# edshkim98/LocalDiffusion-Hallucination

Hardware: AMD Instinct MI355X
Metric: local patches/sec (256^2, T=1000) (higher is better)
Workload: dtype bf16; 1 GPU; cfg3: 8 local patches (vertical band masks) of one 3x256x256 image per GPU, 4-stage dim-32 conditional UNet (12.1M params), DDPM T=1000, pred_x0, sigmoid schedule; patches_per_gpu=8, parallelism=patch-sharded x1, one all-gather per sample, step_graph_replay=True, whole_batch_graph_flag=False, concurrent_sub_batches=2, weight_split_levels=0

## Files before the change

include/localdiff_hip.h:

```cpp
#ifndef LOCALDIFF_HIP_H
#define LOCALDIFF_HIP_H

#include <stddef.h>
#include <stdint.h>

#ifdef __cplusplus
extern "C" {
#endif

#define LD_OK 0
#define LD_EINVAL (-1)
#define LD_EHIP (-2)
#define LD_ETIMEOUT (-3)

#define LD_F32 0
#define LD_BF16 1
#define LD_F16 2

#define LD_STAT_STRIPES 16

#define LD_ACT_NONE 0
#define LD_ACT_SILU 1
#define LD_ACT_RELU 2

// ... 38 lines not shown
  int32_t gn_groups;
  int32_t act;
  const float* film;
  int32_t film_tstride;
  int32_t film_bstride;
} ld_src;

typedef struct ld_conv3x3_args {
  ld_src src[2];
  int32_t nsrc;
  const void* weight;
  const float* bias;
  void* out;
  double* out_stats;
  int32_t out_groups;
  int32_t B, H, W, Cout;
  const int32_t* t_ptr;
  int32_t dtype;
  const void* addend;
  int32_t weight_terms;
  const void* side_weight;
  const float* side_bias;
  void* side_out;
} ld_conv3x3_args;
int ld_conv3x3(const ld_conv3x3_args* args, void* stream);

#define LD_EPI_PLAIN 0
#define LD_EPI_QKV_LINEAR 1
#define LD_EPI_QKV_FULL 2
#define LD_EPI_RMS_RES 3
#define LD_EPI_RES 4
#define LD_EPI_GN_TAIL 5
typedef struct ld_conv1x1_args {
  ld_src src[2];
  int32_t nsrc;
  int32_t unshuffle;
  int32_t rms_in;
  const void* weight;
  int64_t weight_bstride;
  const float* bias;
  int32_t epilogue;
  int32_t hidden;
  float q_scale;
  const float* g2;
  const void* residual;
  ld_src gn_tail;
// ... 429 lines not shown
```

localdiffusion-hallucination_amd/_cabi.py:

```python
import ctypes as C
import os

from .tuning import lib_override_path

_HERE = os.path.dirname(os.path.abspath(__file__))

LIB_PATH = lib_override_path() or os.path.join(_HERE, "csrc", "liblocaldiff_hip.so")

LD_F32, LD_BF16, LD_F16 = 0, 1, 2
ACT_NONE, ACT_SILU, ACT_RELU = 0, 1, 2
EPI_PLAIN, EPI_QKV_LINEAR, EPI_QKV_FULL, EPI_RMS_RES, EPI_RES, EPI_GN_TAIL = 0, 1, 2, 3, 4, 5
OBJ = {"pred_x0": 0, "pred_noise": 1, "pred_v": 2}
SCHED_COLS = 8
STAT_STRIPES = 16
COUNTER_CONV3X3_C32, COUNTER_CONV3X3_GENERIC, COUNTER_CONV3X3_S32 = 0, 1, 2
SEG_SRC_PLAIN, SEG_SRC_POOL, SEG_SRC_CAT_D2S = 0, 1, 2
CLF_PLAIN, CLF_HALVE, CLF_AFFINE = 0, 1, 2

vp, i32, i64, u64, f32 = C.c_void_p, C.c_int32, C.c_int64, C.c_uint64, C.c_float


class Src(C.Structure):
    _fields_ = [("data", vp), ("C", i32), ("pix_stride", i32), ("upsample", i32), ("gn_stats", vp),
                ("gn_gamma", vp), ("gn_beta", vp), ("gn_groups", i32), ("act", i32), ("film", vp),
                ("film_tstride", i32), ("film_bstride", i32)]


class Conv3x3Args(C.Structure):
    _fields_ = [("src", Src * 2), ("nsrc", i32), ("weight", vp), ("bias", vp), ("out", vp),
                ("out_stats", vp), ("out_groups", i32), ("B", i32), ("H", i32), ("W", i32),
                ("Cout", i32), ("t_ptr", vp), ("dtype", i32), ("addend", vp), ("weight_terms", i32),
                ("side_weight", vp), ("side_bias", vp), ("side_out", vp)]


class Conv1x1Args(C.Structure):
    _fields_ = [("src", Src * 2), ("nsrc", i32), ("unshuffle", i32), ("rms_in", i32), ("weight", vp),
                ("weight_bstride", i64), ("bias", vp), ("epilogue", i32), ("hidden", i32),
                ("q_scale", f32), ("g2", vp), ("residual", vp), ("gn_tail", Src), ("out", vp), ("kmax_out", vp), ("B", i32), ("H", i32),
                ("W", i32), ("Cout", i32), ("dtype", i32), ("weight_terms", i32)]


class GnApplyArgs(C.Structure):
    _fields_ = [("a", Src), ("b", Src), ("final_act", i32), ("pool", i32), ("out", vp), ("B", i32),
                ("H", i32), ("W", i32), ("t_ptr", vp), ("dtype", i32)]


class StepBeginArgs(C.Structure):
    _fields_ = [("zero_a", vp), ("bytes_a", C.c_size_t), ("zero_b", vp), ("bytes_b", C.c_size_t), ("t_ptr", vp), ("delta", i32),
                ("idx_ptr", vp), ("t_table", vp), ("film_rows", vp), ("row_floats", i32), ("film_cur", vp)]


class SegConvArgs(C.Structure):
    _fields_ = [("src0", vp), ("src1", vp), ("C0", i32), ("C1", i32), ("mode", i32), ("ksize", i32), ("weight", vp),
                ("scale", vp), ("shift", vp), ("relu", i32), ("out", vp), ("B", i32), ("H", i32), ("W", i32),
                ("Cout", i32), ("dtype", i32)]
# ... 278 lines not shown
```

localdiffusion-hallucination_amd/csrc/conv3x3.hip:

```cpp
#include "common.hip.h"
#include <stdlib.h>

int ld_conv3x3_c32_try(const ld_conv3x3_args* p, hipStream_t st);
int ld_conv3x3_s32_try(const ld_conv3x3_args* p, hipStream_t st);
#ifdef LD_DEBUG_VARIANTS
int ld_conv3x3_ksplit_try(const ld_conv3x3_args* p, hipStream_t st);
int ld_conv3x3_ring_try(const ld_conv3x3_args* p, hipStream_t st);
#endif

#include "conv3x3_body.hip.h"

namespace {

#ifdef LD_DEBUG_VARIANTS
int g_span_shape[1024][5];
#endif

template <typename T, int MT, int NW, bool DEEP, int DBG, bool SK = false, bool RAW = false, bool SIDE = false>
int launch_dbg(const Conv3Dev& a, hipStream_t st) {
  constexpr int TR = 4 * NW, HR = TR + 2, HC = 18;
  constexpr int NPIXP = (HR * HC + 15) / 16 * 16;
  const int ctot = a.s[0].C + (a.nsrc > 1 ? a.s[1].C : 0);
  const size_t lds = (SK ? 2 : 1) * (4 * NPIXP * 16 + (9 + (SIDE ? 1 : 0)) * MT * 1024) + 2 * ctot * sizeof(float) + 4 * 2 * 16 * MT * sizeof(double);
  Conv3Dev d = a;
  d.tiles_x = (a.W + 15) / 16;
  const int tiles_y = (a.H + TR - 1) / TR;
  dim3 grid(d.tiles_x * tiles_y, a.Cout / (16 * MT), a.B);
  if (lds > 65536) LD_HIP(ld_allow_lds(conv3x3_kernel<T, MT, NW, DEEP, DBG, SK, RAW, SIDE>, lds));
  LD_LAUNCH((conv3x3_kernel<T, MT, NW, DEEP, DBG, SK, RAW, SIDE>), grid, dim3(SK ? 512 : 256), lds, st, d.s[0].data, d.w, d.H, d.W, d.tiles_x,
            d.s[0].C, d.s[0].ld, d.s[0].ups, d.nsrc, d.wsplit, d.Cout, d);
  LD_LAUNCH_CHECK("conv3x3");
  return LD_OK;
}

template <typename T, int MT, int NW, bool DEEP>
int launch(const Conv3Dev& a, hipStream_t st) {
#ifdef LD_DEBUG_VARIANTS
  if constexpr (std::is_same<T, bf16>::value && !DEEP) {
    switch (a.dbg & 255) {
      case 1: return launch_dbg<T, MT, NW, DEEP, 1>(a, st);
      case 2: return launch_dbg<T, MT, NW, DEEP, 2>(a, st);
      case 3: return launch_dbg<T, MT, NW, DEEP, 3>(a, st);
      case 4: return launch_dbg<T, MT, NW, DEEP, 4>(a, st);
      case 7: return launch_dbg<T, MT, NW, DEEP, 7>(a, st);
      case 8: return launch_dbg<T, MT, NW, DEEP, 8>(a, st);
      case 12: return launch_dbg<T, MT, NW, DEEP, 12>(a, st);
      case 15: return launch_dbg<T, MT, NW, DEEP, 15>(a, st);
      case 64: return launch_dbg<T, MT, NW, DEEP, 64>(a, st);
      case 128:
        if (!a.s[0].stats && !(a.nsrc > 1 && a.s[1].stats)) return launch_dbg<T, MT, NW, DEEP, 128, false, true>(a, st);
        return launch_dbg<T, MT, NW, DEEP, 128>(a, st);
      default: break;
    }
  }
#endif
  if constexpr (!DEEP) {
    const bool raw = !a.s[0].stats && !(a.nsrc > 1 && a.s[1].stats);
    if (raw && ld_tuning().conv_raw) return launch_dbg<T, MT, NW, DEEP, 0, false, true>(a, st);
  }
  return launch_dbg<T, MT, NW, DEEP, 0>(a, st);
}

template <typename T>
int dispatch(const Conv3Dev& a, hipStream_t st) {
#ifdef LD_DEBUG_VARIANTS
  static const int force_mt = getenv("LD_CONV_MT") ? atoi(getenv("LD_CONV_MT")) : 0;
  static const int force_nw = getenv("LD_CONV_NW") ? atoi(getenv("LD_CONV_NW")) : 0;
#else
  constexpr int force_mt = 0, force_nw = 0;
#endif
  const LdTuning& tn = ld_tuning();
  bool mt4 = (a.Cout % 64) == 0;
  const long mt4_min = tn.conv_mt4_min_wgs;
  if (mt4 && (long)((a.W + 15) / 16) * ((a.H + 7) / 8) * (a.Cout / 64) * a.B < mt4_min) mt4 = false;
  const long blocks16 = (long)((a.W + 15) / 16) * ((a.H + 15) / 16) * (a.Cout / (mt4 ? 64 : 32)) * a.B;
  const long big_min = tn.conv_big_min;
  bool big = blocks16 >= big_min && a.H >= 16 && !mt4;
  if (mt4 && a.H >= 16 && blocks16 >= tn.conv_big4_min) big = true;
  if (force_mt == 2) mt4 = false;
  if (force_mt == 4 && (a.Cout % 64) == 0) mt4 = true;
  if (force_nw == 2) big = false;
  if (force_nw == 4) big = true;
#ifdef LD_DEBUG_VARIANTS
  static const int force_deep = getenv("LD_CONV_DEEP") ? atoi(getenv("LD_CONV_DEEP")) : -1;
#else
  constexpr int force_deep = -1;
#endif
  const int ck = sizeof(T) == 4 ? 16 : 32;
  const int nch = (a.s[0].C + (a.nsrc > 1 ? a.s[1].C : 0)) / ck;
  const long wg = (long)((a.W + 15) / 16) * ((a.H + 7) / 8) * (a.Cout / (mt4 ? 64 : 32)) * a.B;
  bool deep = false;
  if (force_deep >= 0) deep = force_deep != 0;
  if constexpr (sizeof(T) == 2) {
    if (a.w2) {
      if (mt4) return launch_dbg<T, 4, 2, false, 0, false, true, true>(a, st);
      return launch_dbg<T, 2, 2, false, 0, false, true, true>(a, st);
    }
  }
  const int force_sk = (int)tn.conv_sk;
  const long sk_max_wgs = tn.conv_sk_max_wgs;
  bool sk = force_sk >= 1 && sizeof(T) == 2 && !big && !deep && ((nch >= 8 && wg <= sk_max_wgs) || force_sk == 2);
  if constexpr (sizeof(T) == 2) {
    if (sk) return mt4 ? launch_dbg<T, 4, 2, false, 0, true>(a, st) : launch_dbg<T, 2, 2, false, 0, true>(a, st);
  }
#ifdef LD_DEBUG_VARIANTS
  if (deep && !big) return mt4 ? launch<T, 4, 2, true>(a, st) : launch<T, 2, 2, true>(a, st);
#endif
  (void)deep;
  if (mt4) return big ? launch<T, 4, 4, false>(a, st) : launch<T, 4, 2, false>(a, st);
  return big ? launch<T, 2, 4, false>(a, st) : launch<T, 2, 2, false>(a, st);
}

}

#ifdef LD_DEBUG_VARIANTS
extern "C" int ld_debug_conv_spans(unsigned long long* spans, int* shapes) {
  LD_HIP(hipDeviceSynchronize());
// ... 23 lines not shown
    LD_REQUIRE(S.data != nullptr, "ld_conv3x3: src[%d] null", s);
    LD_REQUIRE(S.C > 0 && S.C % 32 == 0, "ld_conv3x3: src[%d].C=%d must be a multiple of 32", s, S.C);
    if (S.upsample) LD_REQUIRE(p->H % 2 == 0 && p->W % 2 == 0, "ld_conv3x3: upsample needs even H,W");
    if (S.gn_stats) {
      LD_REQUIRE(S.gn_groups <= 16, "ld_conv3x3: src[%d] gn_groups %d > 16 (the stripe reduction uses 16 lanes per group)", s, S.gn_groups);
      LD_REQUIRE(S.gn_gamma && S.gn_beta && S.gn_groups > 0 && S.C % S.gn_groups == 0,
                 "ld_conv3x3: src[%d] GroupNorm prologue incomplete", s);
    }
    a.s[s] = to_dev(S);
  }
  if (p->nsrc == 1) a.s[1] = a.s[0];
  if (p->out_stats) {
    LD_REQUIRE(p->out_groups > 0 && p->Cout % p->out_groups == 0 && (p->Cout / p->out_groups) <= 32,
               "ld_conv3x3: out_groups %d incompatible with Cout %d", p->out_groups, p->Cout);
  }
  a.w = p->weight; a.bias = p->bias; a.out = p->out; a.ostats = p->out_stats;
  a.ogroups = p->out_groups > 0 ? p->out_groups : 1;
  a.B = p->B; a.H = p->H; a.W = p->W; a.Cout = p->Cout; a.t_ptr = p->t_ptr; a.tiles_x = 0;
  a.addend = p->addend;
  a.w2 = p->side_weight; a.bias2 = p->side_bias; a.out2 = p->side_out;
  if (p->side_weight) {
    LD_REQUIRE(ld_dtype_16(p->dtype), "ld_conv3x3: the side (res_conv) output needs 16-bit storage");
    LD_REQUIRE(p->side_bias && p->side_out, "ld_conv3x3: side_weight without side_bias / side_out");
    LD_REQUIRE(p->weight_terms != 2 && !p->addend, "ld_conv3x3: the side output does not combine with two-term weights or an addend");
    for (int s = 0; s < p->nsrc; ++s)
      LD_REQUIRE(!p->src[s].gn_stats && !p->src[s].upsample, "ld_conv3x3: the side output needs raw, un-resampled sources (a ResnetBlock's block1)");
  }
  LD_REQUIRE(p->weight_terms >= 0 && p->weight_terms <= 2 && !(p->weight_terms == 2 && !ld_dtype_16(p->dtype)),
             "ld_conv3x3: weight_terms %d (2 needs 16-bit storage)", p->weight_terms);
  a.wsplit = p->weight_terms == 2 ? 1 : 0;
  a.dbg = 0;
#ifdef LD_DEBUG_VARIANTS
  static const int dbg = getenv("LD_CONV_DEBUG") ? atoi(getenv("LD_CONV_DEBUG")) : 0;
  a.dbg = dbg;
  if (dbg == 128) {
    static int calls = 0;
    const int slot = calls++ & 1023;
    g_span_shape[slot][0] = p->B; g_span_shape[slot][1] = p->H; g_span_shape[slot][2] = p->W;
    g_span_shape[slot][3] = p->src[0].C + (p->nsrc > 1 ? p->src[1].C : 0); g_span_shape[slot][4] = p->Cout;
    a.dbg = 128 | (slot << 8);
  }
#endif
  hipStream_t st = reinterpret_cast<hipStream_t>(stream);
  if (p->side_weight) {
    ld_count(LD_COUNTER_CONV3X3_GENERIC);
    return LD_DISPATCH16(p->dtype, dispatch<T>(a, st));
  }
  if (p->weight_terms != 2) {
    const int rc = ld_conv3x3_c32_try(p, st);
    if (rc != 0) return rc < 0 ? rc : LD_OK;
  }
  {
    const int rc = ld_conv3x3_s32_try(p, st);
    if (rc != 0) return rc < 0 ? rc : LD_OK;
  }
#ifdef LD_DEBUG_VARIANTS
  {
    const int rc = ld_conv3x3_ring_try(p, st);
    if (rc != 0) return rc < 0 ? rc : LD_OK;
  }
  static const int ksplit = getenv("LD_CONV_KSPLIT") ? atoi(getenv("LD_CONV_KSPLIT")) : 0;
  if (ksplit && p->weight_terms != 2) {
    const int rc = ld_conv3x3_ksplit_try(p, st);
    if (rc != 0) return rc < 0 ? rc : LD_OK;
  }
#endif
  ld_count(LD_COUNTER_CONV3X3_GENERIC);
  return LD_DISPATCH(p->dtype, dispatch<T>(a, st));
}
// ... 1 lines not shown
```

localdiffusion-hallucination_amd/csrc/conv3x3_body.hip.h:

```cpp
#pragma once
#include "common.hip.h"

namespace {

struct Conv3Dev {
  SrcDev s[2];
  const void* w;
  const float* bias;
  void* out;
  double* ostats;
  const int* t_ptr;
  const void* addend;
  const void* w2;
  const float* bias2;
  void* out2;
  int nsrc;
  int ogroups;
  int B, H, W, Cout;
  int tiles_x;
  int wsplit;
  int dbg;
};

__device__ unsigned long long g_conv_trace[24];
__device__ unsigned long long g_conv_span[1024][2];
#define TR_STAMP(k) do { if ((DBG & 64) && tracing) tr_t[k] = __builtin_readcyclecounter(); } while (0)

typedef const Conv3Dev __attribute__((address_space(4)))* Conv3KernargPtr;
template <typename T, int MT, int NW, bool DEEP, int DBG, bool SK = false, bool RAW = false, bool SIDE = false>
__device__ __forceinline__ void conv3x3_tile(const Conv3Dev& head, Conv3KernargPtr rest, const int bx, const int by, const int bz,
                                             const int gdx, const int gdz, char* smem) {
  Conv3Dev a = head;
  constexpr int E = DT<T>::E, CK = DT<T>::CK;
  constexpr int TR = 4 * NW, TC = 16, HR = TR + 2, HC = TC + 2;
  constexpr int NPIX = HR * HC, NPIXP = (NPIX + 15) / 16 * 16, PLANE = NPIXP * 16;
  constexpr int ITER = (NPIXP + 63) / 64;
  constexpr int UNITS = 9 * MT * 64, WU = (UNITS + 255) / 256;
  constexpr bool P = DT<T>::precise;

  static_assert(!SIDE || (RAW && !SK && !DEEP && MT * NW < 16 && sizeof(T) == 2), "SIDE: RAW 16-bit launches of the small register tiles");
  constexpr int STAGE = 4 * PLANE + (9 + (SIDE ? 1 : 0)) * MT * 1024;
  const int half = SK ? (int)(threadIdx.x >> 8) : 0;
  char* s_x = smem + half * STAGE;
  char* s_w = s_x + 4 * PLANE;
  char* s_w2 = s_w + 9 * MT * 1024;
  float* s_coef = reinterpret_cast<float*>(smem + (SK ? 2 : 1) * STAGE);
  double* s_stat;

  const int tid = threadIdx.x & 255, lane = tid & 63, wv = tid >> 6, px = lane & 15, kq = lane >> 4;
  unsigned long long tr_t[24] = {0};
  const bool tracing = (DBG & 64) && threadIdx.x == 0 && bz == gdz / 2 && by == 0 &&
                       bx == (gdx * 5) / 8;
  TR_STAMP(0);
  if ((DBG & 128) && threadIdx.x == 0 && bx == 0 && by == 0 && bz == 0)
    g_conv_span[(a.dbg >> 8) & 1023][0] = __builtin_amdgcn_s_memrealtime();
  const int b = bz, m0 = by * MT;
  int ty_, tx_;
  tile_of(bx, a.tiles_x, gdx / a.tiles_x, ty_, tx_);
  const int ty0 = ty_ * TR, tx0 = tx_ * TC;
  const int H = a.H, W = a.W;
  const int nch0 = a.s[0].C / CK;
  const int ws = a.wsplit;
  int nch = 0;
// ... 106 lines not shown
        }
        *reinterpret_cast<uint4*>(s_x + kq * PLANE + q * 16) = raw;
      }
    }
  };

  TR_STAMP(1);
  if constexpr (SK) { if (half < nch) issue_loads(half, hxA, wxA, std::false_type{}); }
  else issue_loads(0, hxA, wxA, std::true_type{});
  TR_STAMP(2);
  if (rest) {
    Conv3KernargPtr pr = rest;
    asm volatile("" : "+s"(pr));
    a.s[1].data = pr->s[1].data; a.s[1].stats = pr->s[1].stats; a.s[1].gamma = pr->s[1].gamma; a.s[1].beta = pr->s[1].beta;
    a.s[1].film = pr->s[1].film; a.s[1].C = pr->s[1].C; a.s[1].ld = pr->s[1].ld; a.s[1].ups = pr->s[1].ups;
    a.s[1].groups = pr->s[1].groups; a.s[1].act = pr->s[1].act; a.s[1].film_tstride = pr->s[1].film_tstride;
    a.s[1].film_bstride = pr->s[1].film_bstride;
    a.s[0].stats = pr->s[0].stats; a.s[0].gamma = pr->s[0].gamma; a.s[0].beta = pr->s[0].beta; a.s[0].film = pr->s[0].film;
    a.s[0].groups = pr->s[0].groups; a.s[0].act = pr->s[0].act; a.s[0].film_tstride = pr->s[0].film_tstride;
    a.s[0].film_bstride = pr->s[0].film_bstride;
    a.bias = pr->bias; a.out = pr->out; a.ostats = pr->ostats; a.t_ptr = pr->t_ptr; a.addend = pr->addend;
    a.ogroups = pr->ogroups; a.B = pr->B; a.dbg = pr->dbg;
    if constexpr (SIDE) { a.w2 = pr->w2; a.bias2 = pr->bias2; a.out2 = pr->out2; }
  }
  if constexpr (!SK) second_source();
  {
    const int c1 = a.nsrc > 1 ? a.s[1].C : 0;
    nch = (nch0 + c1 / CK) << ws;
    s_stat = reinterpret_cast<double*>(s_coef + 2 * (a.s[0].C + c1));
  }
  asm volatile("" ::"s"(a.bias), "s"(a.out), "s"(a.ostats), "s"(a.ogroups), "s"(a.addend), "s"(a.s[1].C), "s"(a.s[1].ld), "s"(a.s[1].ups),
               "s"(a.s[1].data), "s"(a.s[0].stats), "s"(a.s[0].gamma), "s"(a.s[0].beta), "s"(a.s[0].film), "s"(a.s[0].groups), "s"(a.s[0].act));
  float4 bias[MT];
#pragma unroll
  for (int m = 0; m < MT; ++m) bias[m] = *reinterpret_cast<const float4*>(a.bias + (m0 + m) * 16 + kq * 4);
  float4 bias2[SIDE ? MT : 1];
  if constexpr (SIDE) {
    asm volatile("" ::"s"(a.w2), "s"(a.bias2), "s"(a.out2));
    if (tid < MT * 64) wx2 = *reinterpret_cast<const uint4*>(reinterpret_cast<const char*>(a.w2) + (long)m0 * 1024 + tid * 16);
#pragma unroll
    for (int m = 0; m < MT; ++m) bias2[m] = *reinterpret_cast<const float4*>(a.bias2 + (m0 + m) * 16 + kq * 4);
  }

  {
    const bool any = !RAW && (a.s[0].stats != nullptr || (a.nsrc > 1 && a.s[1].stats != nullptr));
    if (any) {
// ... 160 lines not shown
        compute();
      }
    }
  }

  const int gx = tx0 + px;
  const long obase = (((long)b * H + ty0) * W + tx0) * a.Cout + m0 * 16;
  char* outb = reinterpret_cast<char*>(a.out) + obase * (long)sizeof(T);
  const char* addb = reinterpret_cast<const char*>(a.addend) + obase * (long)sizeof(T);
  const unsigned lane_off = (__umul24(__umul24(wv * NW, W) + px, a.Cout) + kq * 4) * (unsigned)sizeof(T);
  const unsigned row_off = __umul24(W, a.Cout) * (unsigned)sizeof(T);
  float ssum[MT][4], ssq[MT][4];
#pragma unroll
  for (int m = 0; m < MT; ++m)
#pragma unroll
    for (int r = 0; r < 4; ++r) ssum[m][r] = ssq[m][r] = 0.f;
#pragma unroll
  for (int m = 0; m < MT; ++m) asm volatile("" ::"v"(bias[m].x), "v"(bias[m].y), "v"(bias[m].z), "v"(bias[m].w));
  if constexpr (SIDE) {
#pragma unroll
    for (int m = 0; m < MT; ++m) asm volatile("" ::"v"(bias2[m].x), "v"(bias2[m].y), "v"(bias2[m].z), "v"(bias2[m].w));
  }
  const bool rows_in = ty0 + TR <= H && tx0 + TC <= W;
  auto emit = [&](auto full_tag) {
    constexpr bool FULL = decltype(full_tag)::value;
    typename Raw4<T>::type ad[FULL ? 1 : MT][FULL ? 1 : NW];
    if constexpr (!FULL) {
      if (a.addend) {
#pragma unroll
        for (int m = 0; m < MT; ++m)
#pragma unroll
          for (int j = 0; j < NW; ++j) {
            const int gy = ty0 + wv * NW + j;
            const bool in = rows_in || (gy < H && gx < W);
            const unsigned off = lane_off + j * row_off + m * 16 * (unsigned)sizeof(T);
            ad[m][j] = load4_raw<T>(reinterpret_cast<const T*>(addb + (in ? off : 0u)));
          }
#pragma unroll
        for (int m = 0; m < MT; ++m)
#pragma unroll
          for (int j = 0; j < NW; ++j) pin_raw4(ad[m][j]);
      }
    }
    constexpr int MS = sizeof(T) == 2 ? 2 : 1;
    static_assert(MT % 2 == 0, "m-tiles are stored in pairs");
#pragma unroll
// ... 14 lines not shown
              unpack4<T>(ad[m + mm][j], av);
#pragma unroll
              for (int r = 0; r < 4; ++r) v[mm][r] += av[r];
            }
          }
        }
        if constexpr (MS == 2) {
          const uint4 w16 = pair_frag16<T>(v[0], v[1]);
          const unsigned off = lane_off - kq * 4 * (unsigned)sizeof(T) + j * row_off + m * 16 * (unsigned)sizeof(T) + pair_frag16_off(kq);
          if (valid && !(DBG & 8)) store16_out(outb + off, w16);
        } else {
          const unsigned off = lane_off + j * row_off + m * 16 * (unsigned)sizeof(T);
          if (valid && !(DBG & 8)) store4<T>(reinterpret_cast<T*>(outb + off), v[0]);
        }
        if (valid) {
#pragma unroll
          for (int mm = 0; mm < MS; ++mm)
#pragma unroll
            for (int r = 0; r < 4; ++r) { ssum[m + mm][r] += v[mm][r]; ssq[m + mm][r] += v[mm][r] * v[mm][r]; }
        }
      }
    }
  };
  if (rows_in && !a.addend && half == 0) emit(std::true_type{});
  else emit(std::false_type{});
  if constexpr (SIDE) {
    char* out2b = reinterpret_cast<char*>(a.out2) + obase * (long)sizeof(T);
#pragma unroll
    for (int m = 0; m < MT; m += 2) {
#pragma unroll
      for (int j = 0; j < NW; ++j) {
        const int gy = ty0 + wv * NW + j;
        const bool valid = rows_in || (gy < H && gx < W);
        float v[2][4];
#pragma unroll
        for (int mm = 0; mm < 2; ++mm) {
          const float4 bv = bias2[m + mm];
          v[mm][0] = acc2[m + mm][j][0] + bv.x; v[mm][1] = acc2[m + mm][j][1] + bv.y;
          v[mm][2] = acc2[m + mm][j][2] + bv.z; v[mm][3] = acc2[m + mm][j][3] + bv.w;
        }
        const uint4 w16 = pair_frag16<T>(v[0], v[1]);
        const unsigned off = lane_off - kq * 4 * (unsigned)sizeof(T) + j * row_off + m * 16 * (unsigned)sizeof(T) + pair_frag16_off(kq);
        if (valid) store16_out(out2b + off, w16);
      }
    }
  }
  TR_STAMP(9);
  if (a.ostats) {
    __syncthreads();
    TR_STAMP(16);
    const int gs = a.Cout / a.ogroups;
    const int ngrp_blk = (16 * MT) / gs;
    const int stripe = bx % LD_STAT_STRIPES;
    if (!P && (gs & 3) == 0) {
#pragma unroll
      for (int m = 0; m < MT; ++m) {
        const float s1 = wave16_sum((ssum[m][0] + ssum[m][1]) + (ssum[m][2] + ssum[m][3]));
        const float s2 = wave16_sum((ssq[m][0] + ssq[m][1]) + (ssq[m][2] + ssq[m][3]));
        if (px == 0 && half == 0) {
          s_stat[(wv * 2 + 0) * 4 * MT + m * 4 + kq] = (double)s1;
          s_stat[(wv * 2 + 1) * 4 * MT + m * 4 + kq] = (double)s2;
        }
// ... 39 lines not shown
      if (tid < 2 * ngrp_blk && half == 0) {
        const int gi = tid >> 1, k = tid & 1;
        double acc1 = 0.0;
        for (int w4 = 0; w4 < 4; ++w4)
          for (int c = 0; c < gs; ++c) acc1 += s_stat[(w4 * 2 + k) * 16 * MT + gi * gs + c];
        const int g = (m0 * 16) / gs + gi;
        atomicAdd(&a.ostats[(((size_t)b * LD_STAT_STRIPES + stripe) * a.ogroups + g) * 2 + k], acc1);
      }
    }
  }
  if ((DBG & 128) && threadIdx.x == 0) {
    asm volatile("s_waitcnt vmcnt(0)" ::: "memory");
    atomicMax(&g_conv_span[(a.dbg >> 8) & 1023][1], (unsigned long long)__builtin_amdgcn_s_memrealtime());
  }
  if ((DBG & 64) && tracing) {
    tr_t[19] = __builtin_readcyclecounter();
    asm volatile("s_waitcnt vmcnt(0)" ::: "memory");
    tr_t[10] = __builtin_readcyclecounter();
#pragma unroll
    for (int k = 0; k < 24; ++k) g_conv_trace[k] = tr_t[k];
  }
}

template <typename T, int MT, int NW, bool DEEP, int DBG, bool SK = false, bool RAW = false, bool SIDE = false>
__global__ __launch_bounds__(SK ? 512 : 256) __attribute__((amdgpu_waves_per_eu(SK ? 2 : (MT == 2 ? 3 : 1), SK ? 2 : (MT == 2 ? 3 : 2))))
void conv3x3_kernel(const void* data0, const void* w, int H, int W, int tiles_x, int C0, int ld0, int ups0, int nsrc, int wsplit, int Cout,
                    Conv3Dev rest) {
  extern __shared__ __attribute__((aligned(16))) char smem[];
  Conv3Dev a{};
  a.s[0].data = data0; a.w = w; a.H = H; a.W = W; a.tiles_x = tiles_x; a.s[0].C = C0; a.s[0].ld = ld0; a.s[0].ups = ups0;
  a.nsrc = nsrc; a.wsplit = wsplit; a.Cout = Cout;
  constexpr unsigned REST_OFF = ld_kernarg_offset<const void*, const void*, int, int, int, int, int, int, int, int, int>(alignof(Conv3Dev));
  static_assert(REST_OFF == 56, "conv3x3_kernel: leading arguments changed");
  typedef const char __attribute__((address_space(4)))* KChar;
  Conv3KernargPtr pr = (Conv3KernargPtr)((KChar)__builtin_amdgcn_kernarg_segment_ptr() + REST_OFF);
  if constexpr (SK) {
    a = rest;
    a.tiles_x = tiles_x;
    conv3x3_tile<T, MT, NW, DEEP, DBG, SK, RAW>(a, nullptr, blockIdx.x, blockIdx.y, blockIdx.z, gridDim.x, gridDim.z, smem);
  } else {
    conv3x3_tile<T, MT, NW, DEEP, DBG, SK, RAW, SIDE>(a, pr, blockIdx.x, blockIdx.y, blockIdx.z, gridDim.x, gridDim.z, smem);
  }
}

}
```

localdiffusion-hallucination_amd/unet.py:

```python
import ctypes as C
import math

import numpy as np
import torch
from torch import nn

from . import _cabi as cabi
from .pool import check_declared, intervals_from_declared, peak_live, place_intervals
from .tuning import Tuning
from .weights import UnetConfig, unet_param_shapes

_TORCH_DT = {"fp32": torch.float32, "bf16": torch.bfloat16, "fp16": torch.float16}
_LOWP = ("bf16", "fp16")


def _register(root: nn.Module, dotted: str, tensor: torch.Tensor):
    parts = dotted.split(".")
    mod = root
    for name in parts[:-1]:
        if name not in mod._modules:
            mod.add_module(name, nn.Module())
        mod = mod._modules[name]
    mod.register_parameter(parts[-1], nn.Parameter(tensor, requires_grad=False))

# ... 218 lines not shown
        tn = self.tuning
        key = (B, H, W, table_T, self.compute_dtype, instance, self.weight_split_levels,
               tn.separate_act, tn.sep_act_max_px, tn.sep_act_min_c, tn.fusion_fold, tn.side_res_conv, tn.side_res_conv_max_px, tn.side_res_conv_px, tn.fused_step_begin, tn.linattn_chunk_px, tn.buffer_reuse, tn.recompute_stem, tn.pool_by_size, tn.pool_verify)
        if key not in self._plans:
            self._plans[key] = _Plan(self, B, H, W, table_T)
        return self._plans[key]

    @torch.no_grad()
    def forward(self, x, cond_img, time, x_self_cond=None):
        B, _, H, W = x.shape
        if self.self_condition:
            c = self.cfg.channels
            raise RuntimeError(f"Given groups=1, weight of size [{self.cfg.init_dim}, {c}, 7, 7], expected input[{B}, {2 * c}, {H}, {W}] to have "
                               f"{c} channels, but got {2 * c} channels instead (self_condition=True: ddpm.py:406-413)")
        p = self.plan(B, H, W)
        st = torch.cuda.current_stream().cuda_stream
        p.x_in.copy_(x.to(torch.float32))
        p.cond_in.copy_(cond_img.to(torch.float32))
        p.times.copy_(time.to(torch.int32))
        p.run_time(st)
        p.run_cond(st)
        p.run_main(st)
        return p.model_out.clone()


class _Plan:

    def __init__(self, net: Unet, B, H, W, table_T=None):
        self.net, self.B, self.H, self.W, self.table_T = net, B, H, W, table_T
        self.lib = cabi.lib()
        self.dev = net.device
        self.dt = cabi.dtype_code(net.compute_dtype)
        self.tdt = _TORCH_DT[net.compute_dtype]
        self.esize = 4 if self.dt == cabi.LD_F32 else 2
        self.P = net.packed()
        self.tn = net.tuning
        self.f32 = self.P["f32"]
        cfg = net.cfg
        self.cfg = cfg
        self.keep = []
        self._track = None
        self.named = {}
        self.meta = {}
        self.decl = {}
        self.live_out = []
        self.ops_time, self.ops_cond, self.ops_main = [], [], []
# ... 220 lines not shown
            s.film_tstride = s.film_bstride = 0
        elif film is not None:
            s.film = film.data_ptr()
            s.film_tstride = 0
            s.film_bstride = 2 * c
        self.keep.append(t)
        s._tensor = t
        return s

    def _call(self, ops, fn, args, what, meta=None, reads=(), writes=()):
        self.keep.append(args)
        ref = C.byref(args)
        ops.append(lambda st, fn=fn, ref=ref, what=what: cabi.check(fn(ref, st), what))
        if ops is self.ops_main:
            self.meta[len(ops) - 1] = dict(what=what, **(meta or {}))
            self.decl[len(ops) - 1] = ([t for t in reads if t is not None], [t for t in writes if t is not None])

    def _raw(self, ops, fn, what, nbytes=0, flops=0, reads=(), writes=()):
        ops.append(fn)
        if ops is self.ops_main:
            self.meta[len(ops) - 1] = dict(what=what, family=what, bytes=nbytes, flops=flops)
            self.decl[len(ops) - 1] = ([t for t in reads if t is not None], [t for t in writes if t is not None])

    def conv3(self, ops, srcs, wname, cout, h, w, stats=None, groups=8, weight=None, bias=None, addend=None, side=None):
        a = cabi.Conv3x3Args()
        for i, s in enumerate(srcs):
            a.src[i] = s
        a.nsrc = len(srcs)
        weight = self.P["w"][wname + ".weight"] if weight is None else weight
        bias = self.f32[wname + ".bias"] if bias is None else bias
        a.weight, a.bias = weight.data_ptr(), bias.data_ptr()
        a.weight_terms = 2 if weight.data_ptr() in self.P["terms2"] else 1
        a.addend = cabi.ptr(addend)
        self.keep += [weight, bias, addend]
        out = self.buf(h, w, cout)
        a.out = out.data_ptr()
        side_out = None
        if side is not None:
            side_out = self.buf(h, w, cout)
            a.side_weight, a.side_bias, a.side_out = side[0].data_ptr(), side[1].data_ptr(), side_out.data_ptr()
            self.keep += [side[0], side[1]]
        if stats is not None:
            a.out_stats, a.out_groups = stats.data_ptr(), groups
        a.B, a.H, a.W, a.Cout = self.B, h, w, cout
        a.t_ptr = self.t_ptr()
        a.dtype = self.dt
        cin = sum(s.C for s in srcs)
        npx = self.B * h * w
        mt4 = cout % 64 == 0 and ((w + 15) // 16) * ((h + 7) // 8) * (cout // 64) * self.B >= 256
        blocks16 = ((w + 15) // 16) * ((h + 15) // 16) * (cout // (64 if mt4 else 32)) * self.B
        big = blocks16 >= 512 and h >= 16 and not mt4
        big = big or (mt4 and h >= 16 and blocks16 >= self._kt("conv_big4_min"))
        dname = {cabi.LD_F32: "f32", cabi.LD_BF16: "bf16", cabi.LD_F16: "f16"}[self.dt]
        if side is not None:
            big = False
        fam = f"conv3x3<{dname},{4 if mt4 else 2},{4 if big else 2}>"
        ck = 16 if self.dt == cabi.LD_F32 else 32
        if side is not None:
            pass
        elif (cout == 32 and len(srcs) == 1 and cin == ck and addend is None and h >= 32 and w >= 32 and h % 16 == 0
                and w % 16 == 0 and (w // 16) * (h // 16) * self.B >= self._kt("conv_c32_min_tiles")
                and self._kt("conv_c32") and a.weight_terms != 2):
            fam = f"conv3x3_c32<{dname}>"
        elif (self.dt != cabi.LD_F32 and cout == 32 and addend is None and a.weight_terms != 2 and h % 16 == 0 and w % 16 == 0
              and (w // 16) * (h // 16) * self.B >= self._kt("conv_s32_min_tiles") and not any(s.upsample for s in srcs)
              and cin in (32, 64) and (len(srcs) == 1 or all(s.C == 32 for s in srcs)) and groups in (1, 2, 4, 8)):
            pro = any(s.gn_stats for s in srcs)
            bit = 2 if pro else (1 if cin == 32 else 4)
            if (self._kt("conv_s32") & bit) and (not pro or (len(srcs) == 1 and srcs[0].C == 32 and srcs[0].gn_groups == 8)):
                fam = f"conv3x3_s32<{dname}>"
        in_el = sum(s.C * (npx // 4 if s.upsample else npx) for s in srcs)
        side_b = (in_el + npx * cout + cin * cout) * self.esize + 4 * cout if side is not None else 0
        self._call(ops, self.lib.ld_conv3x3, a, "conv3x3 " + wname + (" + res_conv" if side is not None else ""),
                   dict(family=fam, bytes=(in_el + npx * cout + 9 * cin * cout) * self.esize + 4 * cout + side_b,
                        flops=2 * (9 + (1 if side is not None else 0)) * cin * cout * npx, shape=f"{cin}->{cout}@{h}x{w}"),
                   reads=[s._tensor for s in srcs] + [addend], writes=[out, side_out])
        return out if side is None else (out, side_out)

    def conv1(self, ops, srcs, weight, cout, h, w, bias=None, epi=cabi.EPI_PLAIN, unshuffle=0, rms_in=0,
              bstride=0, g2=None, residual=None, what="conv1x1", out=None, kmax_out=None, gn_tail=None):
        a = cabi.Conv1x1Args()
        for i, s in enumerate(srcs):
            a.src[i] = s
        a.nsrc, a.unshuffle, a.rms_in = len(srcs), unshuffle, rms_in
        a.weight, a.weight_bstride = weight.data_ptr(), bstride
        a.weight_terms = 2 if weight.data_ptr() in self.P["terms2"] else 1
        a.bias = cabi.ptr(bias)
        a.epilogue, a.hidden, a.q_scale = epi, self.cfg.hidden, self.cfg.attn_dim_head ** -0.5
        a.g2, a.residual = cabi.ptr(g2), cabi.ptr(residual)
        a.kmax_out = cabi.ptr(kmax_out)
        if gn_tail is not None:
            a.gn_tail = gn_tail
        out = self.buf(h, w, cout) if out is None else out
        a.out = out.data_ptr()
        a.B, a.H, a.W, a.Cout, a.dtype = self.B, h, w, cout, self.dt
        self.keep += [weight, bias, g2, residual]
        cin = sum(s.C for s in srcs) * (4 if unshuffle else 1)
        npx = self.B * h * w
        el = npx * cin + npx * cout + cin * cout * (self.B if bstride else 1) + (npx * cout if (residual is not None or gn_tail is not None) else 0)
# ... 34 lines not shown
                td, self.temb.data_ptr(), st), "time_mlp (learned Fourier features)"))
        else:
            self.ops_time.append(lambda st: cabi.check(lib.ld_time_mlp(
                times.data_ptr(), n, freqs.data_ptr(), cfg.dim, f["time_mlp.1.weight"].data_ptr(),
                f["time_mlp.1.bias"].data_ptr(), f["time_mlp.3.weight"].data_ptr(), f["time_mlp.3.bias"].data_ptr(),
                td, self.temb.data_ptr(), st), "time_mlp"))
        for name in f:
            if name.endswith(".mlp.1.weight") and not name.startswith("conv_fusion"):
                p = name[:-len(".mlp.1.weight")]
                two_c = f[name].shape[0]
                film = torch.zeros(n, two_c, dtype=torch.float32, device=self.dev)
                self.films[p] = film
                self._film_off[id(film)] = self.film_row
                self.film_row += two_c
                w, b = f[name], f[p + ".mlp.1.bias"]
                self.ops_time.append(lambda st, w=w, b=b, film=film, two_c=two_c: cabi.check(lib.ld_film(
                    self.temb.data_ptr(), n, td, w.data_ptr(), b.data_ptr(), two_c, film.data_ptr(), st), "film"))

    def resnet_block(self, ops, p, srcs_fn, cin_total, cout, h, w, res_tensor=None):
        f, G = self.f32, self.cfg.resnet_block_groups
        s1, s2 = self.slot(), self.slot()
        wres = self.P["w"].get(p + ".res_conv.weight")
        side = None
        px_ok = (h * w in self.tn.side_res_conv_px) if self.tn.side_res_conv_px is not None else h * w <= self.tn.side_res_conv_max_px
        if (wres is not None and self.tn.side_res_conv and self.dt != cabi.LD_F32 and px_ok and self.net.weight_split_levels == 0
                and wres.data_ptr() not in self.P["terms2"] and self.P["w"][p + ".block1.proj.weight"].data_ptr() not in self.P["terms2"]):
            side = (wres, f[p + ".res_conv.bias"])
        rc = None
        if side is not None:
            raw1, rc = self.conv3(ops, srcs_fn(), p + ".block1.proj", cout, h, w, stats=s1, groups=G, side=side)
        else:
            raw1 = self.conv3(ops, srcs_fn(), p + ".block1.proj", cout, h, w, stats=s1, groups=G)
        film = self.films.get(p)
        n1 = self.src(raw1, cout, gn=(s1, f[p + ".block1.norm.weight"], f[p + ".block1.norm.bias"], G),
                      act=cabi.ACT_SILU, film=film)
        if self._separate_act(h * w, cout):
            act1 = self.gn_apply(ops, n1, None, h, w, cout)
            n1 = self.src(act1, cout)
        raw2 = self.conv3(ops, [n1], p + ".block2.proj", cout, h, w, stats=s2, groups=G)
        n2 = self.src(raw2, cout, gn=(s2, f[p + ".block2.norm.weight"], f[p + ".block2.norm.bias"], G),
                      act=cabi.ACT_SILU)
        if rc is not None:
            out = self.gn_apply(ops, n2, self.src(rc, cout), h, w, cout)
        elif (p + ".res_conv.weight") in f:
            out = self.conv1(ops, srcs_fn(), self.P["w"][p + ".res_conv.weight"], cout, h, w,
                             bias=f[p + ".res_conv.bias"], epi=cabi.EPI_GN_TAIL, gn_tail=n2, what="res_conv+tail " + p)
        else:
            assert res_tensor is not None and cin_total == cout
            out = self.gn_apply(ops, n2, self.src(res_tensor, cout), h, w, cout)
        self.named[p] = out
        return out

    def fusion_block_folded(self, ops, x, c, h, w):
        f, G, p = self.f32, self.cfg.resnet_block_groups, "conv_fusion"
        p1, p2, zero = self.fusion_const
        s1, s2 = self.slot(), self.slot()
        raw1 = self.conv3(ops, [self.src(x, c)], p + ".block1.proj", c, h, w, stats=s1, groups=G,
                          weight=self.P["w"][p + ".block1.proj.weight#x"], bias=zero, addend=p1)
        n1 = self.src(raw1, c, gn=(s1, f[p + ".block1.norm.weight"], f[p + ".block1.norm.bias"], G),
                      act=cabi.ACT_SILU, film=self.films.get(p))
        if self._separate_act(h * w, c):
            n1 = self.src(self.gn_apply(ops, n1, None, h, w, c), c)
        raw2 = self.conv3(ops, [n1], p + ".block2.proj", c, h, w, stats=s2, groups=G)
        n2 = self.src(raw2, c, gn=(s2, f[p + ".block2.norm.weight"], f[p + ".block2.norm.bias"], G), act=cabi.ACT_SILU)
        out = self.conv1(ops, [self.src(x, c)], self.P["w"][p + ".res_conv.weight#x"], c, h, w, bias=None,
                         epi=cabi.EPI_GN_TAIL, gn_tail=n2, residual=p2, what="res_conv+tail " + p)
        self.named[p] = out
        return out

    def linear_attention_fused(self, ops, p, x, c, h, w):
        f, cfg, lib = self.f32, self.cfg, self.lib
        n, hid, B, heads, dt, es = h * w, cfg.hidden, self.B, cfg.attn_heads, self.dt, self.esize
        rule = self.tn.chunk_rule(B)
        chunk_px = rule[0] if n >= 65536 else (rule[1] if n >= 16384 else rule[2])
        nchunks = max(1, min(128, n // chunk_px)) if heads == 4 else max(1, min(32, n // 256))
        if heads == 4 and self.tn.linattn_chunk_px is None:
            while B * nchunks < 512 and nchunks < 512 and n // (2 * nchunks) >= 256:
                nchunks *= 2
        ctx = self._tracked(torch.empty(int(lib.ld_linattn_ctx_part_floats(B, heads, 32, nchunks)), dtype=torch.float32, device=self.dev))
        wfold = self._tracked(torch.empty(B, c * hid, dtype=self.tdt, device=self.dev))
        wout = f[p + ".to_out.0.weight"].reshape(c, hid).contiguous()
        wq, wkv = self.P["wq"][p], self.P["wkv"][p]
        kshift = self.P["kshift"].get(p) if heads == 4 else None
        ksp = kshift.data_ptr() if kshift is not None else None
        qshift = self.P["qshift"].get(p) if heads == 4 else None
        qsp = qshift.data_ptr() if qshift is not None else None
        bias, g2 = f[p + ".to_out.0.bias"], self.P["g2"][p + ".to_out.1.g"]
        out = self.buf(h, w, c)
        self.keep += [ctx, wfold, wout, wq, wkv, kshift, qshift, bias, g2, out, x]
# ... 280 lines not shown
```

Baseline: 6.701 patches/s.

## Fuse conv_fusion res_conv into block1 conv3x3 side output with addend; add tall side tile

Adds a side-output addend variant (SADD) to the conv3x3 kernel so conv_fusion's 1x1 res_conv plus its constant residual is computed inside block1's 3x3 launch. The tail then becomes a gn_apply instead of a separate conv1x1 with a GN tail epilogue. It also allows the side res_conv path to use the taller NW=4 tile for larger pixel counts, and adjusts waves_per_eu for that case. Intent is to drop one launch and a re-read of the input, at the cost of more registers held for the extra addend fragments. Route selection now passes px=0 for conv_fusion and reads tuning knobs in the Python mirror.

```diff
diff --git a/include/localdiff_hip.h b/include/localdiff_hip.h
--- a/include/localdiff_hip.h
+++ b/include/localdiff_hip.h
@@ -84,6 +84,8 @@
   const void* side_weight;
   const float* side_bias;
   void* side_out;
+  const void* side_addend;
+  int32_t side_tall;
 } ld_conv3x3_args;
 int ld_conv3x3(const ld_conv3x3_args* args, void* stream);
 
diff --git a/localdiffusion-hallucination_amd/_cabi.py b/localdiffusion-hallucination_amd/_cabi.py
--- a/localdiffusion-hallucination_amd/_cabi.py
+++ b/localdiffusion-hallucination_amd/_cabi.py
@@ -30,7 +30,7 @@
     _fields_ = [("src", Src * 2), ("nsrc", i32), ("weight", vp), ("bias", vp), ("out", vp),
                 ("out_stats", vp), ("out_groups", i32), ("B", i32), ("H", i32), ("W", i32),
                 ("Cout", i32), ("t_ptr", vp), ("dtype", i32), ("addend", vp), ("weight_terms", i32),
-                ("side_weight", vp), ("side_bias", vp), ("side_out", vp)]
+                ("side_weight", vp), ("side_bias", vp), ("side_out", vp), ("side_addend", vp), ("side_tall", i32)]
 
 
 class Conv1x1Args(C.Structure):
diff --git a/localdiffusion-hallucination_amd/csrc/conv3x3.hip b/localdiffusion-hallucination_amd/csrc/conv3x3.hip
--- a/localdiffusion-hallucination_amd/csrc/conv3x3.hip
+++ b/localdiffusion-hallucination_amd/csrc/conv3x3.hip
@@ -16,7 +16,7 @@
 int g_span_shape[1024][5];
 #endif
 
-template <typename T, int MT, int NW, bool DEEP, int DBG, bool SK = false, bool RAW = false, bool SIDE = false>
+template <typename T, int MT, int NW, bool DEEP, int DBG, bool SK = false, bool RAW = false, bool SIDE = false, bool SADD = false>
 int launch_dbg(const Conv3Dev& a, hipStream_t st) {
   constexpr int TR = 4 * NW, HR = TR + 2, HC = 18;
   constexpr int NPIXP = (HR * HC + 15) / 16 * 16;
@@ -26,8 +26,8 @@
   d.tiles_x = (a.W + 15) / 16;
   const int tiles_y = (a.H + TR - 1) / TR;
   dim3 grid(d.tiles_x * tiles_y, a.Cout / (16 * MT), a.B);
-  if (lds > 65536) LD_HIP(ld_allow_lds(conv3x3_kernel<T, MT, NW, DEEP, DBG, SK, RAW, SIDE>, lds));
-  LD_LAUNCH((conv3x3_kernel<T, MT, NW, DEEP, DBG, SK, RAW, SIDE>), grid, dim3(SK ? 512 : 256), lds, st, d.s[0].data, d.w, d.H, d.W, d.tiles_x,
+  if (lds > 65536) LD_HIP(ld_allow_lds(conv3x3_kernel<T, MT, NW, DEEP, DBG, SK, RAW, SIDE, SADD>, lds));
+  LD_LAUNCH((conv3x3_kernel<T, MT, NW, DEEP, DBG, SK, RAW, SIDE, SADD>), grid, dim3(SK ? 512 : 256), lds, st, d.s[0].data, d.w, d.H, d.W, d.tiles_x,
             d.s[0].C, d.s[0].ld, d.s[0].ups, d.nsrc, d.wsplit, d.Cout, d);
   LD_LAUNCH_CHECK("conv3x3");
   return LD_OK;
@@ -62,7 +62,7 @@
 }
 
 template <typename T>
-int dispatch(const Conv3Dev& a, hipStream_t st) {
+int dispatch(const Conv3Dev& a, hipStream_t st, bool side_tall = false, bool side_addend = false) {
 #ifdef LD_DEBUG_VARIANTS
   static const int force_mt = getenv("LD_CONV_MT") ? atoi(getenv("LD_CONV_MT")) : 0;
   static const int force_nw = getenv("LD_CONV_NW") ? atoi(getenv("LD_CONV_NW")) : 0;
@@ -93,6 +93,11 @@
   if (force_deep >= 0) deep = force_deep != 0;
   if constexpr (sizeof(T) == 2) {
     if (a.w2) {
+      if (side_addend) {
+        LD_REQUIRE(!mt4, "ld_conv3x3: the side addend exists on the 32-channel x 8-row tile only (this launch takes a 64-channel tile)");
+        return launch_dbg<T, 2, 2, false, 0, false, true, true, true>(a, st);
+      }
+      if (side_tall && big && !mt4) return launch_dbg<T, 2, 4, false, 0, false, true, true>(a, st);
       if (mt4) return launch_dbg<T, 4, 2, false, 0, false, true, true>(a, st);
       return launch_dbg<T, 2, 2, false, 0, false, true, true>(a, st);
     }
@@ -162,7 +167,8 @@
   if (p->side_weight) {
     LD_REQUIRE(ld_dtype_16(p->dtype), "ld_conv3x3: the side (res_conv) output needs 16-bit storage");
     LD_REQUIRE(p->side_bias && p->side_out, "ld_conv3x3: side_weight without side_bias / side_out");
-    LD_REQUIRE(p->weight_terms != 2 && !p->addend, "ld_conv3x3: the side output does not combine with two-term weights or an addend");
+    LD_REQUIRE(p->weight_terms != 2, "ld_conv3x3: the side output does not combine with two-term weights");
+    LD_REQUIRE(!p->addend || p->side_addend, "ld_conv3x3: a side output beside an addend needs side_addend too (the one variant built: conv_fusion's)");
     for (int s = 0; s < p->nsrc; ++s)
       LD_REQUIRE(!p->src[s].gn_stats && !p->src[s].upsample, "ld_conv3x3: the side output needs raw, un-resampled sources (a ResnetBlock's block1)");
   }
@@ -182,9 +188,11 @@
   }
 #endif
   hipStream_t st = reinterpret_cast<hipStream_t>(stream);
+  LD_REQUIRE(!p->side_addend || p->side_weight, "ld_conv3x3: side_addend without side_weight");
   if (p->side_weight) {
+    if (p->side_addend) a.addend2 = p->side_addend;
     ld_count(LD_COUNTER_CONV3X3_GENERIC);
-    return LD_DISPATCH16(p->dtype, dispatch<T>(a, st));
+    return LD_DISPATCH16(p->dtype, dispatch<T>(a, st, p->side_tall != 0, p->side_addend != nullptr));
   }
   if (p->weight_terms != 2) {
     const int rc = ld_conv3x3_c32_try(p, st);
diff --git a/localdiffusion-hallucination_amd/csrc/conv3x3_body.hip.h b/localdiffusion-hallucination_amd/csrc/conv3x3_body.hip.h
--- a/localdiffusion-hallucination_amd/csrc/conv3x3_body.hip.h
+++ b/localdiffusion-hallucination_amd/csrc/conv3x3_body.hip.h
@@ -9,7 +9,10 @@
   const float* bias;
   void* out;
   double* ostats;
-  const int* t_ptr;
+  union {
+    const int* t_ptr;
+    const void* addend2;
+  };
   const void* addend;
   const void* w2;
   const float* bias2;
@@ -27,7 +30,7 @@
 #define TR_STAMP(k) do { if ((DBG & 64) && tracing) tr_t[k] = __builtin_readcyclecounter(); } while (0)
 
 typedef const Conv3Dev __attribute__((address_space(4)))* Conv3KernargPtr;
-template <typename T, int MT, int NW, bool DEEP, int DBG, bool SK = false, bool RAW = false, bool SIDE = false>
+template <typename T, int MT, int NW, bool DEEP, int DBG, bool SK = false, bool RAW = false, bool SIDE = false, bool SADD = false>
 __device__ __forceinline__ void conv3x3_tile(const Conv3Dev& head, Conv3KernargPtr rest, const int bx, const int by, const int bz,
                                              const int gdx, const int gdz, char* smem) {
   Conv3Dev a = head;
@@ -38,7 +41,8 @@
   constexpr int UNITS = 9 * MT * 64, WU = (UNITS + 255) / 256;
   constexpr bool P = DT<T>::precise;
 
-  static_assert(!SIDE || (RAW && !SK && !DEEP && MT * NW < 16 && sizeof(T) == 2), "SIDE: RAW 16-bit launches of the small register tiles");
+  static_assert(!SIDE || (RAW && !SK && !DEEP && MT * NW < 16 && sizeof(T) == 2), "SIDE: RAW 16-bit launches of the register tiles below 16 fragments");
+  static_assert(!SADD || SIDE, "SADD: an addend of the side output");
   constexpr int STAGE = 4 * PLANE + (9 + (SIDE ? 1 : 0)) * MT * 1024;
   const int half = SK ? (int)(threadIdx.x >> 8) : 0;
   char* s_x = smem + half * STAGE;
@@ -191,6 +195,7 @@
     a.bias = pr->bias; a.out = pr->out; a.ostats = pr->ostats; a.t_ptr = pr->t_ptr; a.addend = pr->addend;
     a.ogroups = pr->ogroups; a.B = pr->B; a.dbg = pr->dbg;
     if constexpr (SIDE) { a.w2 = pr->w2; a.bias2 = pr->bias2; a.out2 = pr->out2; }
+    if constexpr (SADD) a.addend2 = pr->addend2;
   }
   if constexpr (!SK) second_source();
   {
@@ -397,6 +402,23 @@
     for (int m = 0; m < MT; ++m) asm volatile("" ::"v"(bias2[m].x), "v"(bias2[m].y), "v"(bias2[m].z), "v"(bias2[m].w));
   }
   const bool rows_in = ty0 + TR <= H && tx0 + TC <= W;
+  typename Raw4<T>::type ad2[SADD ? MT : 1][SADD ? NW : 1];
+  if constexpr (SADD) {
+    const char* add2b = reinterpret_cast<const char*>(a.addend2) + obase * (long)sizeof(T);
+#pragma unroll
+    for (int m = 0; m < MT; ++m)
+#pragma unroll
+      for (int j = 0; j < NW; ++j) {
+        const int gy = ty0 + wv * NW + j;
+        const bool in = rows_in || (gy < H && gx < W);
+        const unsigned off = lane_off + j * row_off + m * 16 * (unsigned)sizeof(T);
+        ad2[m][j] = load4_raw<T>(reinterpret_cast<const T*>(add2b + (in ? off : 0u)));
+      }
+#pragma unroll
+    for (int m = 0; m < MT; ++m)
+#pragma unroll
+      for (int j = 0; j < NW; ++j) pin_raw4(ad2[m][j]);
+  }
   auto emit = [&](auto full_tag) {
     constexpr bool FULL = decltype(full_tag)::value;
     typename Raw4<T>::type ad[FULL ? 1 : MT][FULL ? 1 : NW];
@@ -457,7 +479,7 @@
       }
     }
   };
-  if (rows_in && !a.addend && half == 0) emit(std::true_type{});
+  if (!SADD && rows_in && !a.addend && half == 0) emit(std::true_type{});
   else emit(std::false_type{});
   if constexpr (SIDE) {
     char* out2b = reinterpret_cast<char*>(a.out2) + obase * (long)sizeof(T);
@@ -473,6 +495,12 @@
           const float4 bv = bias2[m + mm];
           v[mm][0] = acc2[m + mm][j][0] + bv.x; v[mm][1] = acc2[m + mm][j][1] + bv.y;
           v[mm][2] = acc2[m + mm][j][2] + bv.z; v[mm][3] = acc2[m + mm][j][3] + bv.w;
+          if constexpr (SADD) {
+            float av[4];
+            unpack4<T>(ad2[m + mm][j], av);
+#pragma unroll
+            for (int r = 0; r < 4; ++r) v[mm][r] += av[r];
+          }
         }
         const uint4 w16 = pair_frag16<T>(v[0], v[1]);
         const unsigned off = lane_off - kq * 4 * (unsigned)sizeof(T) + j * row_off + m * 16 * (unsigned)sizeof(T) + pair_frag16_off(kq);
@@ -558,8 +586,10 @@
   }
 }
 
-template <typename T, int MT, int NW, bool DEEP, int DBG, bool SK = false, bool RAW = false, bool SIDE = false>
-__global__ __launch_bounds__(SK ? 512 : 256) __attribute__((amdgpu_waves_per_eu(SK ? 2 : (MT == 2 ? 3 : 1), SK ? 2 : (MT == 2 ? 3 : 2))))
+constexpr int conv3_waves(bool sk, int mt, int nw, bool side, bool hi) { return sk || (side && nw == 4) ? 2 : (mt == 2 ? 3 : (hi ? 2 : 1)); }
+template <typename T, int MT, int NW, bool DEEP, int DBG, bool SK = false, bool RAW = false, bool SIDE = false, bool SADD = false>
+__global__ __launch_bounds__(SK ? 512 : 256)
+__attribute__((amdgpu_waves_per_eu(conv3_waves(SK, MT, NW, SIDE, false), conv3_waves(SK, MT, NW, SIDE, true))))
 void conv3x3_kernel(const void* data0, const void* w, int H, int W, int tiles_x, int C0, int ld0, int ups0, int nsrc, int wsplit, int Cout,
                     Conv3Dev rest) {
   extern __shared__ __attribute__((aligned(16))) char smem[];
@@ -575,7 +605,7 @@
     a.tiles_x = tiles_x;
     conv3x3_tile<T, MT, NW, DEEP, DBG, SK, RAW>(a, nullptr, blockIdx.x, blockIdx.y, blockIdx.z, gridDim.x, gridDim.z, smem);
   } else {
-    conv3x3_tile<T, MT, NW, DEEP, DBG, SK, RAW, SIDE>(a, pr, blockIdx.x, blockIdx.y, blockIdx.z, gridDim.x, gridDim.z, smem);
+    conv3x3_tile<T, MT, NW, DEEP, DBG, SK, RAW, SIDE, SADD>(a, pr, blockIdx.x, blockIdx.y, blockIdx.z, gridDim.x, gridDim.z, smem);
   }
 }
 
diff --git a/localdiffusion-hallucination_amd/unet.py b/localdiffusion-hallucination_amd/unet.py
--- a/localdiffusion-hallucination_amd/unet.py
+++ b/localdiffusion-hallucination_amd/unet.py
@@ -264,6 +264,13 @@
         p.run_cond(st)
         p.run_main(st)
         return p.model_out.clone()
+
+
+def side_res_conv_route(tn, px, sixteen_bit, weight_split_levels):
+    if not (tn.side_res_conv and sixteen_bit and weight_split_levels == 0):
+        return False, False
+    ok = (px in tn.side_res_conv_px) if tn.side_res_conv_px is not None else 0 < px <= tn.side_res_conv_max_px
+    return ok, ok and px > tn.side_res_conv_max_px
 
 
 class _Plan:
@@ -530,7 +537,8 @@
             self.meta[len(ops) - 1] = dict(what=what, family=what, bytes=nbytes, flops=flops)
             self.decl[len(ops) - 1] = ([t for t in reads if t is not None], [t for t in writes if t is not None])
 
-    def conv3(self, ops, srcs, wname, cout, h, w, stats=None, groups=8, weight=None, bias=None, addend=None, side=None):
+    def conv3(self, ops, srcs, wname, cout, h, w, stats=None, groups=8, weight=None, bias=None, addend=None, side=None,
+              side_addend=None, side_tall=False):
         a = cabi.Conv3x3Args()
         for i, s in enumerate(srcs):
             a.src[i] = s
@@ -547,7 +555,8 @@
         if side is not None:
             side_out = self.buf(h, w, cout)
             a.side_weight, a.side_bias, a.side_out = side[0].data_ptr(), side[1].data_ptr(), side_out.data_ptr()
-            self.keep += [side[0], side[1]]
+            a.side_addend, a.side_tall = cabi.ptr(side_addend), int(side_tall)
+            self.keep += [side[0], side[1], side_addend]
         if stats is not None:
             a.out_stats, a.out_groups = stats.data_ptr(), groups
         a.B, a.H, a.W, a.Cout = self.B, h, w, cout
@@ -555,12 +564,12 @@
         a.dtype = self.dt
         cin = sum(s.C for s in srcs)
         npx = self.B * h * w
-        mt4 = cout % 64 == 0 and ((w + 15) // 16) * ((h + 7) // 8) * (cout // 64) * self.B >= 256
+        mt4 = cout % 64 == 0 and ((w + 15) // 16) * ((h + 7) // 8) * (cout // 64) * self.B >= self._kt("conv_mt4_min_wgs")
         blocks16 = ((w + 15) // 16) * ((h + 15) // 16) * (cout // (64 if mt4 else 32)) * self.B
-        big = blocks16 >= 512 and h >= 16 and not mt4
+        big = blocks16 >= self._kt("conv_big_min") and h >= 16 and not mt4
         big = big or (mt4 and h >= 16 and blocks16 >= self._kt("conv_big4_min"))
         dname = {cabi.LD_F32: "f32", cabi.LD_BF16: "bf16", cabi.LD_F16: "f16"}[self.dt]
-        if side is not None:
+        if side is not None and not (side_tall and big and not mt4):
             big = False
         fam = f"conv3x3<{dname},{4 if mt4 else 2},{4 if big else 2}>"
         ck = 16 if self.dt == cabi.LD_F32 else 32
@@ -582,7 +591,7 @@
         self._call(ops, self.lib.ld_conv3x3, a, "conv3x3 " + wname + (" + res_conv" if side is not None else ""),
                    dict(family=fam, bytes=(in_el + npx * cout + 9 * cin * cout) * self.esize + 4 * cout + side_b,
                         flops=2 * (9 + (1 if side is not None else 0)) * cin * cout * npx, shape=f"{cin}->{cout}@{h}x{w}"),
-                   reads=[s._tensor for s in srcs] + [addend], writes=[out, side_out])
+                   reads=[s._tensor for s in srcs] + [addend, side_addend], writes=[out, side_out])
         return out if side is None else (out, side_out)
 
     def conv1(self, ops, srcs, weight, cout, h, w, bias=None, epi=cabi.EPI_PLAIN, unshuffle=0, rms_in=0,
@@ -663,13 +672,13 @@
         s1, s2 = self.slot(), self.slot()
         wres = self.P["w"].get(p + ".res_conv.weight")
         side = None
-        px_ok = (h * w in self.tn.side_res_conv_px) if self.tn.side_res_conv_px is not None else h * w <= self.tn.side_res_conv_max_px
-        if (wres is not None and self.tn.side_res_conv and self.dt != cabi.LD_F32 and px_ok and self.net.weight_split_levels == 0
+        px_ok, tall = side_res_conv_route(self.tn, h * w, self.dt != cabi.LD_F32, self.net.weight_split_levels)
+        if (wres is not None and px_ok
                 and wres.data_ptr() not in self.P["terms2"] and self.P["w"][p + ".block1.proj.weight"].data_ptr() not in self.P["terms2"]):
             side = (wres, f[p + ".res_conv.bias"])
         rc = None
         if side is not None:
-            raw1, rc = self.conv3(ops, srcs_fn(), p + ".block1.proj", cout, h, w, stats=s1, groups=G, side=side)
+            raw1, rc = self.conv3(ops, srcs_fn(), p + ".block1.proj", cout, h, w, stats=s1, groups=G, side=side, side_tall=tall)
         else:
             raw1 = self.conv3(ops, srcs_fn(), p + ".block1.proj", cout, h, w, stats=s1, groups=G)
         film = self.films.get(p)
@@ -696,16 +705,26 @@
         f, G, p = self.f32, self.cfg.resnet_block_groups, "conv_fusion"
         p1, p2, zero = self.fusion_const
         s1, s2 = self.slot(), self.slot()
-        raw1 = self.conv3(ops, [self.src(x, c)], p + ".block1.proj", c, h, w, stats=s1, groups=G,
-                          weight=self.P["w"][p + ".block1.proj.weight#x"], bias=zero, addend=p1)
+        wx1, wres = self.P["w"][p + ".block1.proj.weight#x"], self.P["w"][p + ".res_conv.weight#x"]
+        px_ok, _ = side_res_conv_route(self.tn, 0, self.dt != cabi.LD_F32, self.net.weight_split_levels)
+        small_tile = not (c % 64 == 0 and ((w + 15) // 16) * ((h + 7) // 8) * (c // 64) * self.B >= self._kt("conv_mt4_min_wgs"))
+        rc = None
+        if (px_ok and small_tile and wres.data_ptr() not in self.P["terms2"] and wx1.data_ptr() not in self.P["terms2"]):
+            raw1, rc = self.conv3(ops, [self.src(x, c)], p + ".block1.proj", c, h, w, stats=s1, groups=G, weight=wx1, bias=zero,
+                                  addend=p1, side=(wres, zero), side_addend=p2)
+        else:
+            raw1 = self.conv3(ops, [self.src(x, c)], p + ".block1.proj", c, h, w, stats=s1, groups=G, weight=wx1, bias=zero, addend=p1)
         n1 = self.src(raw1, c, gn=(s1, f[p + ".block1.norm.weight"], f[p + ".block1.norm.bias"], G),
                       act=cabi.ACT_SILU, film=self.films.get(p))
         if self._separate_act(h * w, c):
             n1 = self.src(self.gn_apply(ops, n1, None, h, w, c), c)
         raw2 = self.conv3(ops, [n1], p + ".block2.proj", c, h, w, stats=s2, groups=G)
         n2 = self.src(raw2, c, gn=(s2, f[p + ".block2.norm.weight"], f[p + ".block2.norm.bias"], G), act=cabi.ACT_SILU)
-        out = self.conv1(ops, [self.src(x, c)], self.P["w"][p + ".res_conv.weight#x"], c, h, w, bias=None,
-                         epi=cabi.EPI_GN_TAIL, gn_tail=n2, residual=p2, what="res_conv+tail " + p)
+        if rc is not None:
+            out = self.gn_apply(ops, n2, self.src(rc, c), h, w, c)
+        else:
+            out = self.conv1(ops, [self.src(x, c)], wres, c, h, w, bias=None,
+                             epi=cabi.EPI_GN_TAIL, gn_tail=n2, residual=p2, what="res_conv+tail " + p)
         self.named[p] = out
         return out
 
```

After: 6.561 patches/s. 2.1% lower.
